# rishikksh20/FastSpeech2

Hardware: AMD Instinct MI355X
Metric: mel-frames/sec (higher is better)
Workload: dtype bf16x3 (FFN conv: f16 x f16 + block-scaled e4m3 cross terms; the decoder's: block-scaled e2m1 cross terms, one E8M0 scale per 16-channel block on both operands); 1 GPU; c3: batch=64 LJSpeech-shape; default.yaml dims, free-running, random-init weights (seed 0), duration bias calibrated to 7.87 frames/phoneme; precision=mix_mx4, utterances=64, phonemes=4528, parallelism=single GPU, launch=eager, device-driven layout (no host sync), overlap_encoder=False, streams=3

## Files before the change

### fastspeech2_amd/csrc/fs2_runtime.hip

```cpp
#include <hip/hip_runtime.h>
#include <dlfcn.h>

#include <algorithm>
#include <cmath>
#include <cstdarg>
#include <cstdio>
#include <cstring>
#include <fstream>
#include <iterator>
#include <list>
#include <map>
#include <string>
#include <type_traits>
#include <vector>

#include "../../include/fs2.h"
#include "attn_bf16.h"
#include "attn_w32.h"
#include "attn_f32.h"
#include "attn_plan.h"
#include "common.h"
#include "elementwise.h"
#include "varshort.h"
#include "layout_rule.h"
#include "layout.h"
#include "gemm_bf16.h"
#include "gemm_plan.h"
#include "gemm_planes.h"
#include "gemm_row4.h"
#include "model_launches.h"
#include "call_plan.h"
#include "gemm_mx.h"
#include "weight_plan.h"
#include "gemm_f32.h"
#include "griffin_lim.h"
#include "gl_pitch.h"
// ... 67 lines not shown
    if (!rf) return false;
    const std::string rec((std::istreambuf_iterator<char>(rf)), std::istreambuf_iterator<char>());
    const size_t k = rec.find("\"so_sha16\"");
    if (k == std::string::npos) return false;
    const size_t q0 = rec.find('"', rec.find(':', k) + 1), q1 = q0 == std::string::npos ? q0 : rec.find('"', q0 + 1);
    if (q1 == std::string::npos) return false;
    const std::string want = rec.substr(q0 + 1, q1 - q0 - 1);
    const size_t c = rec.find("\"clean\"");
    const size_t v = c == std::string::npos ? c : rec.find_first_not_of(" :", c + 7);
    if (v == std::string::npos || rec.compare(v, 4, "true") != 0) return false;
    std::ifstream sf(so, std::ios::binary);
    if (!sf) return false;
    Sha256 sh;
    std::vector<unsigned char> blk(1 << 20);
    while (sf) {
        sf.read(reinterpret_cast<char*>(blk.data()), (std::streamsize)blk.size());
        if (sf.gcount() > 0) sh.update(blk.data(), (size_t)sf.gcount());
    }
    return sh.hex16() == want;
}
bool audit_clean() {
    static const bool ok = audit_clean_of_this_binary();
    return ok;
}

Options& opts() {
    static Options o = [] {
        Options x;
        x.bm = env_int("FS2_BM", -1); x.row8 = env_int("FS2_ROW8", -1); x.qkv8 = env_int("FS2_QKV8", -1);
        x.nosplitk = env_int("FS2_NOSPLITK", 0) != 0; x.f32_rows = env_int("FS2_F32_ROWS", 0) != 0; x.mt8 = env_int("FS2_MT8", -1); x.qkv_split = env_int("FS2_QKV_SPLIT", -1); x.op_att_planes = env_int("FS2_OP_ATT_PLANES", 0); x.fuse_var = env_int("FS2_FUSE_VAR", 1); x.bal = env_int("FS2_BAL", 0); x.w32 = env_int("FS2_ATTN_W32", -1);
        x.row4 = env_int("FS2_ROW4", -1); x.mt4 = env_int("FS2_MT4", -1); x.ffn2_mx = env_int("FS2_FFN2_MX", 1); x.qkv4 = env_int("FS2_QKV4", -1); x.post_mx = env_int("FS2_POST_MX", 1);
        x.tokproj = env_int("FS2_TOKPROJ", 3) & 3; x.tokproj_f32 = env_int("FS2_TOKPROJ_F32", 0) != 0;
        x.varshort = env_int("FS2_VARSHORT", 1) != 0;
        if (!audit_clean()) {
            x.w32 = 0; x.row4 = 0; x.qkv4 = 0;
            fprintf(stderr, "libfs2_hip: no clean ISA-audit record of this binary (libfs2_hip.audit.json next to it): attn_w32 and gemm_row4_bf16 are switched "
                            "off, attn_bf16 / gemm_row8_bf16 run instead; rebuild with `python -c 'import __graft_entry__ as g; g.build()'`\n");
        }
        return x;
    }();
    return o;
}

__global__ void row_l1_bound_kernel(const float* w, const float* b, int N, int K, float xmax, unsigned* out) {
    const int n = blockIdx.x;
    float s = 0.f;
    for (int k = threadIdx.x; k < K; k += blockDim.x) s += fabsf(w[(size_t)n * K + k]);
    for (int o = 32; o > 0; o >>= 1) s += __shfl_xor(s, o);
    __shared__ float part[4];
    if ((threadIdx.x & 63) == 0) part[threadIdx.x >> 6] = s;
    __syncthreads();
    if (threadIdx.x == 0) atomicMax(out, __float_as_uint((part[0] + part[1] + part[2] + part[3]) * xmax + (b ? fabsf(b[n]) : 0.f)));
}
float device_row_l1_bound(hipStream_t s, const float* w, const float* b, int N, int K, float xmax, unsigned* scratch) {
    hipMemsetAsync(scratch, 0, 4, s);
    hipLaunchKernelGGL(row_l1_bound_kernel, dim3(N), dim3(256), 0, s, w, b, N, K, xmax, scratch);
    unsigned u = 0;
    hipMemcpyAsync(&u, scratch, 4, hipMemcpyDeviceToHost, s);
    hipStreamSynchronize(s);
    float f;
    memcpy(&f, &u, 4);
    return f;
}

__global__ void absmax_kernel(const float* x, int64_t n, unsigned* out) {
    float m = 0.f;
// ... 102 lines not shown
inline void allow_lds(const void* kernel, size_t bytes, LdsAttr& st) {
    int dev = 0;
    hipGetDevice(&dev);
    bool& d = st.done[dev & 31];
    if (!d) { hipFuncSetAttribute(kernel, hipFuncAttributeMaxDynamicSharedMemorySize, (int)bytes); d = true; }
}

static_assert(kPlanErrArg == FS2_ERR_ARG && kPlanErrHip == FS2_ERR_HIP && kPlanErrState == FS2_ERR_STATE && kPlanErrUnsupported == FS2_ERR_UNSUPPORTED &&
              kPlanFp32 == FS2_PREC_FP32 && kPlanBf16x3 == FS2_PREC_BF16X3 && kPlanMaxHalo == kMaxHalo && kPlanBN == kB16BN && kPrecMixF16x2 == FS2_PREC_MIX_F16X2 &&
              kPrecMixF16x1 == FS2_PREC_MIX_F16X1 && kPrecMixMx == FS2_PREC_MIX_MX && kPrecMixMx4 == FS2_PREC_MIX_MX4, "gemm_plan.h and model_launches.h restate these");

template <auto K, class A>
hipError_t launch_kernel(dim3 grid, dim3 block, size_t lds, hipStream_t s, const A& a, size_t lds_max = 0) {
    static LdsAttr attr;
    allow_lds(reinterpret_cast<const void*>(K), lds_max ? lds_max : lds, attr);
    hipLaunchKernelGGL(K, grid, block, lds, s, a);
    return hipGetLastError();
}
template <int V> using Int = std::integral_constant<int, V>;
template <int V, int... Vs, typename F>
hipError_t pick(int v, F&& f) {
    if (v == V) return f(Int<V>{});
    if constexpr (sizeof...(Vs) > 0) return pick<Vs...>(v, f);
    else return hipErrorInvalidValue;
}
#define CV(x) decltype(x)::value
constexpr int row4_variant(int epi, int arith, int res) { return epi * 100 + arith * 10 + res; }

template <int NSPLIT, int BM, bool K1, int ARITH>
hipError_t launch_pl(hipStream_t s, const GemmArgs& a, size_t extra_lds = 0) {
    dim3 grid((a.N + kB16BN - 1) / kB16BN, ((a.qk_hi ? a.Rvt : a.R) + BM - 1) / BM, a.ksplit > 1 ? a.ksplit : 1);
    return launch_kernel<gemm_pl_bf16<NSPLIT, BM, K1, ARITH>>(grid, dim3(256), pl_lds_bytes<BM, K1>() + extra_lds, s, a);
}
template <int MT, int EPI, int ARITH, int RES>
hipError_t launch_row4(hipStream_t s, const GemmArgs& a) {
    return launch_kernel<gemm_row4_bf16<3, 3, MT, EPI, 2, ARITH, RES>>(dim3((a.R + 32 * MT - 1) / (32 * MT)), dim3(256), row4_lds_bytes<3, MT>(), s, a);
}

hipError_t run_plan(hipStream_t s, const GemmPlan& p, const GemmArgs& t) {
    switch (p.kernel) {
    case GemmKernel::Row4: {
        auto row4 = [&](auto EPI, auto ARITH, auto RES) { return pick<5, 4>(p.mt, [&](auto MT) { return launch_row4<CV(MT), CV(EPI), CV(ARITH), CV(RES)>(s, t); }); };
        switch (row4_variant(p.epi, p.arith, p.res)) {
        case row4_variant(2, 0, 3): return row4(Int<2>{}, Int<0>{}, Int<3>{});
        case row4_variant(1, 0, 1): return row4(Int<1>{}, Int<0>{}, Int<1>{});
        case row4_variant(4, 0, 1): return row4(Int<4>{}, Int<0>{}, Int<1>{});
        case row4_variant(0, 2, 2): return row4(Int<0>{}, Int<2>{}, Int<2>{});
        case row4_variant(0, 0, 2): return row4(Int<0>{}, Int<0>{}, Int<2>{});
        case row4_variant(0, 0, 1): return row4(Int<0>{}, Int<0>{}, Int<1>{});
        }
        break;
    }
    case GemmKernel::Qkv4:
        return pick<5, 4>(p.mt, [&](auto MT) {
            static_assert((size_t)32 * CV(MT) * kQkvLd * 4 <= row4_lds_bytes<3, CV(MT)>(), "the V pass transposes its tile through the operand ring's memory");
            return launch_kernel<gemm_row4_bf16<3, 3, CV(MT), 3, 2, 0>>(dim3((t.Rvt + 32 * CV(MT) - 1) / (32 * CV(MT)), 3), dim3(256), row4_lds_bytes<3, CV(MT)>(), s, t);
        });
    case GemmKernel::PlMx:
        return pick<160, 192, 224, 256, 128, 64>(p.bm, [&](auto BM) { return launch_pl<1, CV(BM), false, 2>(s, t); });
    case GemmKernel::PlMx4:
        return launch_pl<1, 256, false, 3>(s, t, kMx4RowScaleLds + 2048);
    case GemmKernel::PlF16:
        return pick<3, 2, 1>(p.nsplit, [&](auto NS) {
            return pick<256, 128, 64>(p.bm, [&](auto BM) { return launch_pl<CV(NS), CV(BM), false, 1>(s, t); });
        });
    case GemmKernel::Qkv8:
        return pick<3, 2>(p.nb, [&](auto NB) {
            return pick<3, 1>(p.nsplit, [&](auto NS) {
                return pick<3, 2>(p.mt, [&](auto MT) {
                    return pick<1, 0>(p.apart, [&](auto AP) {
                        const dim3 grid((t.Rvt + 64 * CV(MT) - 1) / (64 * CV(MT)), CV(AP) ? 3 : 1);
                        return launch_kernel<gemm_qkv8_bf16<CV(NS), CV(NB), CV(MT), CV(AP) != 0>>(grid, dim3(512), qkv8_lds_bytes<CV(NB), CV(MT)>(), s, t);
                    });
                });
            });
        });
    case GemmKernel::Row8cTwoLn:
        return pick<3, 1>(p.nsplit, [&](auto NS) { return launch_kernel<gemm_row8c_bf16<CV(NS), 4, 2, 2>>(dim3((t.R + 127) / 128, 1), dim3(512), row8c_lds_bytes<4, 2>(), s, t); });
    case GemmKernel::Row8c:
    case GemmKernel::Row8cGrouped:
        return pick<3, 2>(p.nb, [&](auto NB) {
            return pick<3, 1>(p.nsplit, [&](auto NS) {
                return pick<3, 2>(p.mt, [&](auto MT) {
                    const dim3 grid((t.R + 64 * CV(MT) - 1) / (64 * CV(MT)), t.k_groups > 1 ? t.k_groups : 1);
                    return launch_kernel<gemm_row8c_bf16<CV(NS), CV(NB), CV(MT), 1>>(grid, dim3(512), row8c_lds_bytes<CV(NB), CV(MT)>(), s, t);
                });
            });
        });
    case GemmKernel::Row8:
        return pick<3, 2>(p.nb, [&](auto NB) {
            return pick<3, 1>(p.nsplit, [&](auto NS) {
                return pick<3, 2>(p.mt, [&](auto MT) {
                    const dim3 grid((t.R + 64 * CV(MT) - 1) / (64 * CV(MT)));
// ... 1434 lines not shown

int fs2_op_duration(void* stream, const float* d_log, int64_t n, int64_t* d) {
    if (!d_log || !d || n < 0) return fail(nullptr, FS2_ERR_ARG, "fs2_op_duration: bad arguments");
    if (n == 0) return FS2_OK;
    hipLaunchKernelGGL(duration_kernel, dim3((unsigned)((n + 255) / 256)), dim3(256), 0, (hipStream_t)stream, d_log, n, d);
    hipError_t e = hipGetLastError();
    if (e != hipSuccess) return fail(nullptr, FS2_ERR_HIP, "duration: %s", hipGetErrorString(e));
    return FS2_OK;
}

int fs2_set_option(const char* name, int32_t value) {
    if (!name) return fail(nullptr, FS2_ERR_ARG, "fs2_set_option: null name");
    Options& o = opts();
    const std::string n = name;
    if (n == "FS2_BM") o.bm = value;
    else if (n == "FS2_ROW8") o.row8 = value;
    else if (n == "FS2_QKV8") o.qkv8 = value;
    else if (n == "FS2_NOSPLITK") o.nosplitk = value > 0;
    else if (n == "FS2_F32_ROWS") o.f32_rows = value > 0;
    else if (n == "FS2_MT8") o.mt8 = value;
    else if (n == "FS2_QKV_SPLIT") o.qkv_split = value;
    else if (n == "FS2_OP_ATT_PLANES") o.op_att_planes = value;
    else if (n == "FS2_FUSE_VAR") o.fuse_var = value != 0;
    else if (n == "FS2_BAL") o.bal = value < 0 ? 0 : value;
    else if (n == "FS2_ATTN_W32") o.w32 = value;
    else if (n == "FS2_ROW4") o.row4 = value;
    else if (n == "FS2_MT4") o.mt4 = value;
    else if (n == "FS2_FFN2_MX") o.ffn2_mx = value != 0;
    else if (n == "FS2_QKV4") o.qkv4 = value;
    else if (n == "FS2_POST_MX") o.post_mx = value != 0;
    else if (n == "FS2_TOKPROJ") o.tokproj = value < 0 ? 3 : (value & 3);
    else if (n == "FS2_TOKPROJ_F32") o.tokproj_f32 = value > 0;
    else if (n == "FS2_VARSHORT") o.varshort = value != 0;
    else return fail(nullptr, FS2_ERR_ARG, "fs2_set_option: unknown option %s", name);
    return FS2_OK;
}

int fs2_get_option(const char* name, int32_t* value) {
    if (!name || !value) return fail(nullptr, FS2_ERR_ARG, "fs2_get_option: null argument");
    const Options& o = opts();
    const std::string n = name;
    if (n == "FS2_AUDIT_CLEAN") *value = audit_clean() ? 1 : 0;
    else if (n == "attn_w32_active") *value = o.w32 != 0;
    else if (n == "row4_active") *value = o.row4 != 0;
    else if (n == "qkv4_active") *value = o.qkv4 != 0 && o.row4 != 0;
    else if (n == "FS2_BM") *value = o.bm;
    else if (n == "FS2_ROW8") *value = o.row8;
    else if (n == "FS2_QKV8") *value = o.qkv8;
    else if (n == "FS2_NOSPLITK") *value = o.nosplitk;
    else if (n == "FS2_F32_ROWS") *value = o.f32_rows;
    else if (n == "FS2_MT8") *value = o.mt8;
    else if (n == "FS2_QKV_SPLIT") *value = o.qkv_split;
    else if (n == "FS2_OP_ATT_PLANES") *value = o.op_att_planes;
    else if (n == "FS2_FUSE_VAR") *value = o.fuse_var;
    else if (n == "FS2_BAL") *value = o.bal;
    else if (n == "FS2_ATTN_W32") *value = o.w32;
    else if (n == "FS2_ROW4") *value = o.row4;
    else if (n == "FS2_MT4") *value = o.mt4;
    else if (n == "FS2_FFN2_MX") *value = o.ffn2_mx;
    else if (n == "FS2_QKV4") *value = o.qkv4;
    else if (n == "FS2_POST_MX") *value = o.post_mx;
    else if (n == "FS2_TOKPROJ") *value = o.tokproj;
    else if (n == "FS2_TOKPROJ_F32") *value = o.tokproj_f32;
    else if (n == "FS2_VARSHORT") *value = o.varshort;
    else return fail(nullptr, FS2_ERR_ARG, "fs2_get_option: unknown option %s", name);
    return FS2_OK;
}

int fs2_get_counter(fs2_handle* h, void* stream, const char* name, int64_t* value, int32_t reset) {
    if (!h || !name || !value) return fail(h, FS2_ERR_ARG, "fs2_get_counter: null argument");
    if (std::string(name) != "attn_slow_path_waves") return fail(h, FS2_ERR_ARG, "fs2_get_counter: unknown counter %s", name);
    DeviceGuard g(h->cfg.device);
    HIP_TRY(h, g.err);
    hipStream_t s = (hipStream_t)stream;
    int v = 0;
    HIP_TRY(h, hipMemcpyAsync(&v, h->counters, sizeof(int), hipMemcpyDeviceToHost, s));
    if (reset) HIP_TRY(h, hipMemsetAsync(h->counters, 0, sizeof(int), s));
    HIP_TRY(h, hipStreamSynchronize(s));
    *value = v;
    return FS2_OK;
}

int fs2_op_bucketize(void* stream, const float* x, int64_t n, const float* bins, int32_t nb, int32_t* idx) {
    if (!x || !bins || !idx || n < 0) return fail(nullptr, FS2_ERR_ARG, "fs2_op_bucketize: bad arguments");
    if (n == 0) return FS2_OK;
    hipLaunchKernelGGL(bucketize_kernel, dim3((unsigned)((n + 255) / 256)), dim3(256), 0, (hipStream_t)stream, x, n, bins, nb, idx);
    hipError_t e = hipGetLastError();
    if (e != hipSuccess) return fail(nullptr, FS2_ERR_HIP, "bucketize: %s", hipGetErrorString(e));
    return FS2_OK;
}

size_t fs2_op_vocode_workspace_bytes(int32_t B, const int32_t* lens) { return fs2_op_vocode_workspace_bytes_geom(kGlNfft, kGlHop, kGlNfft, 80, B, lens); }

size_t fs2_op_vocode_workspace_bytes_geom(int32_t n_fft, int32_t hop, int32_t win, int32_t n_mels, int32_t B, const int32_t* lens) {
    return gl_workspace_bytes({"fs2_op_vocode_workspace_bytes_geom", GlKind::Synthesis, {n_fft, hop, win, n_mels}, gl_host_batch(B, nullptr, lens)});
}

// ... 208 lines not shown
```

### fastspeech2_amd/csrc/gemm_plan.h

```cpp
#pragma once
#include <algorithm>

#include "gemm_args.h"

namespace fs2 {

constexpr int kPlanErrArg = -1, kPlanErrHip = -2, kPlanErrState = -3, kPlanErrUnsupported = -6;
constexpr int kPlanFp32 = 0, kPlanBf16x3 = 1;
constexpr int kPlanMaxHalo = 16;
constexpr int kPlanBN = 128;

struct Options {
    int bm = -1;
    int bal = 0;
    int row8 = -1;
    int qkv8 = -1;
    int nosplitk = 0;
    int f32_rows = 0;
    int fuse_var = 1;
    int mt8 = -1;
    int op_att_planes = 0;
    int qkv_split = -1;
    int w32 = -1;
    int row4 = -1;
    int mt4 = -1;
    int qkv4 = -1;
    int ffn2_mx = 1;
    int post_mx = 1;
    int tokproj = 3;
    int tokproj_f32 = 0;
    int varshort = 1;
};

constexpr int kSplitRegime = 8192, kSplitRows = 16384;
constexpr int kCus = 256;

inline bool row_regime(long regime_rows, int forced) { return forced >= 0 ? forced != 0 : (regime_rows + 127) / 128 >= 128; }

inline long rows_in_use(const GemmArgs& a, long rows) { return a.regime_rows > 0 ? std::min<long>(rows, a.regime_rows) : rows; }

inline int row8_mt(long rows, int wgs = 1) {
    const long t128 = (rows + 127) / 128, t192 = (rows + 191) / 192;
    if (t128 > kCus && t192 <= kCus) return 3;
    return (wgs > 1 && t128 * wgs > kCus && t192 * wgs <= kCus) ? 3 : 2;
}

inline int row4_mt(long rows) {
    const long r4 = ((rows + 127) / 128 + kCus - 1) / kCus * 128, r5 = ((rows + 159) / 160 + kCus - 1) / kCus * 160;
    return r5 <= r4 ? 5 : 4;
}
inline int row4_epi(const GemmArgs& a) {
    if (a.ktaps != 1 || a.N != 384 || !a.ln_g || a.Y || !a.Yp || a.resid || a.relu_pre || a.dot_w || a.k_groups > 1 || a.ln_groups > 1 || a.qk_hi || a.yp_col_off) return -1;
    if (a.Cpad % 64 != 0 || a.yp_chunks * 32 != a.N) return -1;
    if (a.residp && a.residp_chunks * 32 != a.N) return -1;
    if (a.pe) return (a.act_post == 1 && a.yp_f16 == 0 && !a.residp) ? 2 : -1;
    if (a.act_post != 0 || !a.residp) return -1;
    if (a.yp_f16 == 2) return a.residp_mx ? -1 : 1;
    if (a.yp_f16 == 3) return (a.residp_mx || !a.yp_rowscale) ? -1 : 4;
    return a.yp_f16 == 0 ? 0 : -1;
}

inline void qkv8_plan(long rows, const Options& o, int& mt, int& apart) {
    double best = 1e30;
    for (int m = 2; m <= 3; ++m)
// ... 12 lines not shown
}

inline bool use_qkv8(const GemmArgs& a, const Options& o) {
    if (!a.qk_hi || a.ktaps != 1 || (a.att_D != 256 && a.att_D != 384) || a.N != 3 * a.att_D) return false;
    return row_regime(a.regime_rows ? a.regime_rows : a.Rvt, o.qkv8);
}

inline bool use_row8(const GemmArgs& a, const Options& o) {
    const int Ng = a.k_groups > 1 ? a.N / a.k_groups : a.N;
    const bool two_ln_groups = a.ln_groups == 2 && a.k_groups <= 1 && a.N == 512 && a.ktaps > 1;
    if (a.qk_hi || (!two_ln_groups && Ng != 256 && Ng != 384)) return false;
    if (a.ln_groups > 1 && !two_ln_groups && a.ln_groups != a.k_groups) return false;
    if (a.ktaps > 1) {
        if (!a.ln_g || a.pe || a.f16_terms) return false;
    } else if (a.dot_w || !(a.ln_g || a.pe) || a.k_groups > 1 || a.ln_groups > 1) return false;
    return row_regime(a.regime_rows ? a.regime_rows : a.R, o.row8);
}

inline int conv_bm_balanced(long rows, long nN) {
    const long ypr = std::max<long>(1, 2 * kCus / nN);
    const long rounds = std::max<long>(1, (rows + 256 * ypr - 1) / (256 * ypr));
    const long h = (rows + rounds * ypr - 1) / (rounds * ypr);
    return (int)std::min<long>(256, std::max<long>(160, (h + 31) / 32 * 32));
}
inline int conv_bm(const GemmArgs& a, int arith, int nsplit, int ksplit, const Options& o) {
    const int force = o.bm > 0 ? o.bm : 0;
    const long rows = a.R, nN = (a.N + kPlanBN - 1) / kPlanBN;
    int bm = force ? force : (nN * ((rows + 255) / 256) >= 512 ? 256 : (nN * ((rows + 127) / 128) >= 400 ? 128 : 64));
    if (arith == 1) return bm == 256 ? 256 : (bm == 128 ? 128 : 64);
    if (bm <= 128) return bm == 128 ? 128 : 64;
    if (arith == 0 && nsplit != 3) return 256;
    if (!force && o.bal && (arith == 2 || ksplit <= 1)) bm = conv_bm_balanced(o.bal == 2 ? rows : rows_in_use(a, rows), nN);
    return bm <= 160 ? 160 : (bm <= 192 ? 192 : (bm <= 224 ? 224 : 256));
}

inline int pick_ksplit(const GemmArgs& a, long rr, int max_extra_splits, bool own_y, size_t ld) {
    const int nchunks = a.Cpad / 32;
    const long wgs = (long)((a.N + kPlanBN - 1) / kPlanBN) * ((rr + 63) / 64);
    for (int cand = 4; cand >= 2; --cand)
        if (nchunks % cand == 0 && (nchunks / cand) * a.ktaps >= 4 && wgs * cand <= 1024 && cand - 1 <= max_extra_splits &&
            (size_t)(cand - (own_y ? 1 : 0)) * a.R * ld <= a.kpart_cap) return cand;
    return 1;
}

inline bool rows_supported(int N) { return N == 80 || N == 256 || N == 384; }

enum class GemmKernel {
    None,
    RowsF32,
    TileF32,
    TileRowsF32,
    PlBf16,
    PlF16,
    PlMx,
    PlMx4,
    Row8,
    Row8c,
    Row8cGrouped,
    Row8cTwoLn,
    Row4,
    Qkv8,
    Qkv4,
};
enum class RowsOut { None, Y, Scratch, KpartSlab };

struct GemmPlan {
    GemmKernel kernel = GemmKernel::None;
    int nsplit = 0, nb = 0;
    int bm = 0, mt = 0;
    bool k1 = false;
    int apart = 0, epi = -1, arith = 0, res = 0;
    int ksplit = 1;
    RowsOut y = RowsOut::None;
    bool build_planes = false;
    bool rows_pass = false;
    int err = 0;
    const char* msg = nullptr;
    int m0 = 0, m1 = 0;
    int tile_rows() const { return bm ? bm : (kernel == GemmKernel::Row4 || kernel == GemmKernel::Qkv4 ? 32 : 64) * mt; }
};
inline GemmPlan refused(int err, const char* msg, int m0 = 0, int m1 = 0) {
    GemmPlan p;
    p.err = err; p.msg = msg; p.m0 = m0; p.m1 = m1;
    return p;
}

inline GemmPlan plan_gemm(const GemmArgs& a, int precision, const Options& o) {
    if (a.ktaps - 1 > kPlanMaxHalo) return refused(kPlanErrUnsupported, "%s: kernel size %d > %d", a.ktaps, kPlanMaxHalo + 1);
    if (a.C % 4 != 0 || a.ldx % 4 != 0) return refused(kPlanErrUnsupported, "%s: channels %d / ld %d must be multiples of 4", a.C, a.ldx);
    const bool need_rows = a.ln_g || a.dot_w || a.pe;
    GemmPlan p;
    if (precision == kPlanFp32) {
        if (need_rows && a.N >= 128 && a.N <= 1024 && a.N % 4 == 0 && (a.Y || a.scratch) && !o.f32_rows) {
            p.kernel = GemmKernel::TileRowsF32; p.rows_pass = true;
            p.y = a.Y ? RowsOut::Y : RowsOut::Scratch;
        } else if (need_rows || (a.N < 128 && rows_supported(a.N))) {
            if (!rows_supported(a.N)) return refused(kPlanErrUnsupported, "%s: row-epilogue GEMM needs N in {80,256,384}, got %d", a.N);
            p.kernel = GemmKernel::RowsF32; p.nb = a.N == 80 ? 5 : (a.N == 256 ? 16 : 24);
            p.y = a.Y ? RowsOut::Y : RowsOut::None;
        } else {
            p.kernel = GemmKernel::TileF32; p.y = RowsOut::Y;
        }
        return p;
// ... 7 lines not shown
    const int epi = (row8 && x3 && o.row4 != 0) ? row4_epi(a) : -1;
    if ((a.residp || (need_rows && !a.Y && a.Yp && !a.dot_w && a.ktaps == 1 && !a.scratch)) && epi < 0)
        return refused(kPlanErrState, "%s: a planes-only launch (residual as planes / no fp32 rows) exists on gemm_row4_bf16 only and this one would not run there");
    if (a.yp_col_off && !(row8 && a.ktaps > 1)) return refused(kPlanErrUnsupported, "%s: a plane column offset exists in the row-complete conv kernel only");
    if (a.Yp && a.yp_chunks * 32 >= a.N + 32 && !(row8 && a.ktaps > 1))
        return refused(kPlanErrUnsupported, "%s: planes %d columns wide from a launch of %d: filling a slice of a plane row exists in the row-complete conv kernel only", a.yp_chunks * 32, a.N);
    const bool y_needed = (need_rows && !row8) || (!a.Yp && !a.qk_hi && !(row8 && a.dot_w));
    p.y = a.Y ? RowsOut::Y : ((y_needed && a.scratch) ? RowsOut::Scratch : RowsOut::None);
    if (y_needed && p.y == RowsOut::None) return refused(kPlanErrArg, "%s: no output or scratch buffer");
    if (a.qk_hi && (a.ktaps != 1 || a.att_D % kPlanBN != 0 || a.N != 3 * a.att_D)) return refused(kPlanErrUnsupported, "%s: fused QKV split needs D %% 128 == 0");
    const long rr = a.regime_rows ? a.regime_rows : a.R;
    if (!row8 && !a.qk_hi && a.kpart && !o.nosplitk && a.N <= 1024 && rr <= kSplitRegime && a.R <= kSplitRows && a.mx != 2) {
        const bool own_y = p.y != RowsOut::None;
        p.ksplit = pick_ksplit(a, rr, a.ksplit, own_y, p.y == RowsOut::Y ? (size_t)a.ldy : (size_t)a.N);
        if (p.ksplit > 1 && !own_y) p.y = RowsOut::KpartSlab;
    }
    p.rows_pass = (need_rows && !row8) || p.ksplit > 1;
    const bool mx_row4 = a.mx && a.ktaps == 1 && epi == 0 && a.Cpad % 128 == 0 && a.Xp;
    if ((a.f16_terms || a.mx) && !mx_row4 && (a.ktaps == 1 || need_rows || a.qk_hi)) return refused(kPlanErrUnsupported, "%s: the fp16 arithmetic exists for plain convolutions only");
    if (a.mx && !mx_row4 && (a.ktaps < 3 || a.C % 128 != 0 || a.N % 128 != 0)) return refused(kPlanErrUnsupported, "%s: the mx arithmetic needs a convolution with C %% 128 == 0 and N %% 128 == 0");
    if (a.mx == 2 && (!a.x_rowscale || !a.w_rowscale || !a.Xp || p.ksplit > 1)) return refused(kPlanErrState, "%s: the mx4 arithmetic needs mx4 planes with their row scales and the weight image's channel scales");
    p.build_planes = !a.Xp;
    p.nsplit = x3 ? 3 : 1;
    const int mt8 = (o.mt8 > 0 ? o.mt8 : row8_mt(rows_in_use(a, a.R), a.k_groups > 1 ? a.k_groups : 1)) >= 3 ? 3 : 2;
    const bool force_mt4 = o.mt4 == 4 || o.mt4 == 5;
    if (mx_row4 || epi >= 0) {
        if (a.mx && !a.residp_mx) return refused(kPlanErrHip, "%s launch: invalid argument");
        p.kernel = GemmKernel::Row4; p.epi = epi; p.arith = a.mx ? 2 : 0;
        p.res = epi == 2 ? 3 : ((epi == 0 && a.residp_mx) ? 2 : 1);
        p.mt = force_mt4 ? o.mt4 : row4_mt(rows_in_use(a, a.R));
    } else if (a.mx == 2) {
        if (a.Cpad != 384) return refused(kPlanErrHip, "%s launch: invalid argument");
        p.kernel = GemmKernel::PlMx4; p.nsplit = 1; p.arith = 3; p.bm = 256;
    } else if (a.mx) {
        p.kernel = GemmKernel::PlMx; p.nsplit = 1; p.arith = 2; p.bm = conv_bm(a, 2, 1, p.ksplit, o);
    } else if (a.f16_terms) {
        p.kernel = GemmKernel::PlF16; p.nsplit = a.f16_terms == 3 ? 3 : (a.f16_terms == 2 ? 2 : 1); p.arith = 1; p.bm = conv_bm(a, 1, p.nsplit, p.ksplit, o);
    } else if (use_qkv8(a, o)) {
        if (x3 && o.qkv4 != 0 && o.row4 != 0 && a.att_D == 384 && a.Cpad % 64 == 0) {
            p.kernel = GemmKernel::Qkv4; p.epi = 3; p.mt = force_mt4 ? o.mt4 : qkv4_mt(rows_in_use(a, a.Rvt));
        } else {
            p.kernel = GemmKernel::Qkv8; p.nb = a.att_D == 384 ? 3 : 2; p.mt = 2;
            qkv8_plan(rows_in_use(a, a.Rvt), o, p.mt, p.apart);
        }
    } else if (row8 && a.ktaps > 1 && a.ln_groups == 2 && a.k_groups <= 1) {
        p.kernel = GemmKernel::Row8cTwoLn; p.nb = 4; p.mt = 2;
    } else if (row8 && a.ktaps > 1) {
        p.kernel = a.k_groups > 1 ? GemmKernel::Row8cGrouped : GemmKernel::Row8c;
        p.nb = (a.k_groups > 1 ? a.N / a.k_groups : a.N) == 384 ? 3 : 2; p.mt = mt8;
    } else if (row8) {
        p.kernel = GemmKernel::Row8; p.nb = a.N == 384 ? 3 : 2; p.mt = mt8;
    } else {
        p.kernel = GemmKernel::PlBf16; p.k1 = a.ktaps == 1;
        p.bm = p.k1 ? (o.bm == 128 ? 128 : 64)
                    : conv_bm(a, 0, p.nsplit, p.ksplit, o);
    }
    return p;
}

}
```

### fastspeech2_amd/csrc/gemm_planes.h

```cpp
#pragma once
#include <type_traits>
#include "gemm_bf16.h"

namespace fs2 {

template <int BM, bool K1> constexpr int pl_arows() { return K1 ? BM : BM + kMaxHalo; }
template <int BM, bool K1>
constexpr size_t pl_lds_bytes() {
    const size_t ops = (size_t)(K1 ? 2 : 1) * pl_arows<BM, K1>() * 128 + 2 * (size_t)kB16BN * 128;
    const size_t out = (K1 && BM <= 128) ? (size_t)BM * kQkvLd * 4 : 0;
    return ops > out ? ops : out;
}
typedef __attribute__((address_space(3))) const unsigned short lds_u16_t;
constexpr int kMx4ScLd = 24;
constexpr int kMx4RowScaleLds = 272 * kMx4ScLd;
template <int BM, bool K1> constexpr int pl_occ() { return pl_lds_bytes<BM, K1>() > 53 * 1024 ? 2 : 3; }

__global__ void to_planes(const float* __restrict__ X, int ldx, int C, int R, int nchunks, void* __restrict__ Xp, int f16 = 0, float scale = 1.f) {
    const int64_t i = (int64_t)blockIdx.x * blockDim.x + threadIdx.x;
    const int per_row = nchunks * 8;
    if (i >= (int64_t)R * per_row) return;
    const int row = (int)(i / per_row), c = (int)(i - (int64_t)row * per_row) * 4;
    f32x4 v = f32x4{0.f, 0.f, 0.f, 0.f};
    if (c < C) v = *reinterpret_cast<const f32x4*>(X + (size_t)row * ldx + c);
// ... 275 lines not shown
                    uint2 hi, lo;
                    split4(f32x4{acc[mt][0][r], acc[mt][1][r], acc[mt][2][r], acc[mt][3][r]} * f, hi, lo);
                    const size_t off = (size_t)row * 2 * a.att_D + col;
                    *reinterpret_cast<uint2*>(qkh + off) = hi;
                    *reinterpret_cast<uint2*>(qkl + off) = lo;
                }
            return;
        }
        if (a.qk_hi != nullptr) {
            float* tile = reinterpret_cast<float*>(smem_p);
            __syncthreads();
#pragma unroll
            for (int mt = 0; mt < MT; ++mt)
#pragma unroll
                for (int r = 0; r < 4; ++r)
                {
                    const int trow = wm * (BM / 2) + mt * 16 + rperm(lg * 4 + r);
                    *reinterpret_cast<f32x4*>(tile + trow * kQkvLd + ((wn * 64 + 4 * lr) ^ qkv_tile_swz(trow))) =
                        f32x4{acc[mt][0][r], acc[mt][1][r], acc[mt][2][r], acc[mt][3][r]};
                }
            __syncthreads();
            vt_tile_store<BM>(a, tile, m0, n0, tid);
            return;
        }
    }
    if (ks > 0) {
        GemmArgs p = a;
        p.Y = a.kpart + (size_t)(ks - 1) * a.kpart_stride;
        p.Yp = nullptr; p.relu_pre = 0; p.act_post = 0;
        pl_epilogue<MT>(p, acc, m0 + wm * (BM / 2), col, lg);
        return;
    }
    pl_epilogue<MT>(a, acc, m0 + wm * (BM / 2), col, lg);
}

}

namespace fs2 {

template <int NSPLIT, int MT, int NT>
__device__ __forceinline__ void row8_mfma_step(const char* Bs, int nrow, int lg, const bf16x8_t (&ah)[MT], const bf16x8_t (&al)[MT], f32x4 (&acc)[MT][NT]) {
    constexpr int kReads = NSPLIT == 3 ? 4 : 2, kMfma = 2 * MT * NSPLIT;
    const char* bp0 = Bs + swz(nrow, lg);
    const char* bp1 = Bs + swz(nrow, 4 + lg);
    bf16x8_t bh[2][2], bl[2][2];
#pragma unroll
    for (int u = 0; u < 2; ++u) {
        bh[0][u] = *reinterpret_cast<const bf16x8_t*>(bp0 + u * 2048);
        if (NSPLIT == 3) bl[0][u] = *reinterpret_cast<const bf16x8_t*>(bp1 + u * 2048);
    }
    __builtin_amdgcn_sched_group_barrier(0x100, kReads, 0);
#pragma unroll
    for (int n2 = 0; n2 < NT; n2 += 2) {
        const int cb = (n2 >> 1) & 1, nb = cb ^ 1;
        if (n2 + 2 < NT) {
#pragma unroll
            for (int u = 0; u < 2; ++u) {
                bh[nb][u] = *reinterpret_cast<const bf16x8_t*>(bp0 + (n2 + 2 + u) * 2048);
                if (NSPLIT == 3) bl[nb][u] = *reinterpret_cast<const bf16x8_t*>(bp1 + (n2 + 2 + u) * 2048);
            }
            __builtin_amdgcn_sched_group_barrier(0x100, kReads, 0);
        }
        __builtin_amdgcn_sched_group_barrier(0x008, kMfma, 0);
        if (NSPLIT == 3) {
#pragma unroll
            for (int u = 0; u < 2; ++u)
// ... 585 lines not shown
```

Before: 10.29 million mel-frames/s.

## Add paired-tile MX conv GEMM kernel sharing weight stages across two row tiles

```diff
diff --git a/fastspeech2_amd/csrc/fs2_runtime.hip b/fastspeech2_amd/csrc/fs2_runtime.hip
--- a/fastspeech2_amd/csrc/fs2_runtime.hip
+++ b/fastspeech2_amd/csrc/fs2_runtime.hip
@@ -2,6 +2,7 @@
 #include <dlfcn.h>
 
 #include <algorithm>
+#include <atomic>
 #include <cmath>
 #include <cstdarg>
 #include <cstdio>
@@ -135,6 +136,7 @@
         x.row4 = env_int("FS2_ROW4", -1); x.mt4 = env_int("FS2_MT4", -1); x.ffn2_mx = env_int("FS2_FFN2_MX", 1); x.qkv4 = env_int("FS2_QKV4", -1); x.post_mx = env_int("FS2_POST_MX", 1);
         x.tokproj = env_int("FS2_TOKPROJ", 3) & 3; x.tokproj_f32 = env_int("FS2_TOKPROJ_F32", 0) != 0;
         x.varshort = env_int("FS2_VARSHORT", 1) != 0;
+        x.conv_pair = env_int("FS2_CONV_PAIR", -1);
         if (!audit_clean()) {
             x.w32 = 0; x.row4 = 0; x.qkv4 = 0;
             fprintf(stderr, "libfs2_hip: no clean ISA-audit record of this binary (libfs2_hip.audit.json next to it): attn_w32 and gemm_row4_bf16 are switched "
@@ -303,6 +305,13 @@
     dim3 grid((a.N + kB16BN - 1) / kB16BN, ((a.qk_hi ? a.Rvt : a.R) + BM - 1) / BM, a.ksplit > 1 ? a.ksplit : 1);
     return launch_kernel<gemm_pl_bf16<NSPLIT, BM, K1, ARITH>>(grid, dim3(256), pl_lds_bytes<BM, K1>() + extra_lds, s, a);
 }
+std::atomic<int> g_conv_pair_launches{0};
+template <int ARITH>
+hipError_t launch_pair(hipStream_t s, const GemmArgs& a) {
+    const int tiles = (a.R + 255) / 256;
+    g_conv_pair_launches.fetch_add(1, std::memory_order_relaxed);
+    return launch_kernel<gemm_pl_pair<ARITH>>(dim3((a.N + kB16BN - 1) / kB16BN, (tiles + 1) / 2), dim3(512), pl_pair_lds_bytes<ARITH>(), s, a);
+}
 template <int MT, int EPI, int ARITH, int RES>
 hipError_t launch_row4(hipStream_t s, const GemmArgs& a) {
     return launch_kernel<gemm_row4_bf16<3, 3, MT, EPI, 2, ARITH, RES>>(dim3((a.R + 32 * MT - 1) / (32 * MT)), dim3(256), row4_lds_bytes<3, MT>(), s, a);
@@ -328,8 +337,10 @@
             return launch_kernel<gemm_row4_bf16<3, 3, CV(MT), 3, 2, 0>>(dim3((t.Rvt + 32 * CV(MT) - 1) / (32 * CV(MT)), 3), dim3(256), row4_lds_bytes<3, CV(MT)>(), s, t);
         });
     case GemmKernel::PlMx:
+        if (p.pair) return launch_pair<2>(s, t);
         return pick<160, 192, 224, 256, 128, 64>(p.bm, [&](auto BM) { return launch_pl<1, CV(BM), false, 2>(s, t); });
     case GemmKernel::PlMx4:
+        if (p.pair) return launch_pair<3>(s, t);
         return launch_pl<1, 256, false, 3>(s, t, kMx4RowScaleLds + 2048);
     case GemmKernel::PlF16:
         return pick<3, 2, 1>(p.nsplit, [&](auto NS) {
@@ -1830,6 +1841,7 @@
     else if (n == "FS2_TOKPROJ") o.tokproj = value < 0 ? 3 : (value & 3);
     else if (n == "FS2_TOKPROJ_F32") o.tokproj_f32 = value > 0;
     else if (n == "FS2_VARSHORT") o.varshort = value != 0;
+    else if (n == "FS2_CONV_PAIR") o.conv_pair = value;
     else return fail(nullptr, FS2_ERR_ARG, "fs2_set_option: unknown option %s", name);
     return FS2_OK;
 }
@@ -1861,6 +1873,8 @@
     else if (n == "FS2_TOKPROJ") *value = o.tokproj;
     else if (n == "FS2_TOKPROJ_F32") *value = o.tokproj_f32;
     else if (n == "FS2_VARSHORT") *value = o.varshort;
+    else if (n == "FS2_CONV_PAIR") *value = o.conv_pair;
+    else if (n == "conv_pair_launches") *value = g_conv_pair_launches.load(std::memory_order_relaxed);
     else return fail(nullptr, FS2_ERR_ARG, "fs2_get_option: unknown option %s", name);
     return FS2_OK;
 }
diff --git a/fastspeech2_amd/csrc/gemm_plan.h b/fastspeech2_amd/csrc/gemm_plan.h
--- a/fastspeech2_amd/csrc/gemm_plan.h
+++ b/fastspeech2_amd/csrc/gemm_plan.h
@@ -30,6 +30,7 @@
     int tokproj = 3;
     int tokproj_f32 = 0;
     int varshort = 1;
+    int conv_pair = -1;
 };
 
 constexpr int kSplitRegime = 8192, kSplitRows = 16384;
@@ -108,6 +109,12 @@
     if (arith == 0 && nsplit != 3) return 256;
     if (!force && o.bal && (arith == 2 || ksplit <= 1)) bm = conv_bm_balanced(o.bal == 2 ? rows : rows_in_use(a, rows), nN);
     return bm <= 160 ? 160 : (bm <= 192 ? 192 : (bm <= 224 ? 224 : 256));
+}
+
+inline bool conv_pair_regime(long regime_rows, long nN) { return nN * (((regime_rows + 255) / 256 + 1) / 2) >= kCus; }
+inline bool conv_pair(const GemmArgs& a, int arith, int bm, int ksplit, const Options& o) {
+    if (o.conv_pair == 0 || (arith != 2 && arith != 3) || bm != 256 || ksplit != 1 || a.ktaps <= 1 || a.k_groups > 1 || a.qk_hi) return false;
+    return o.conv_pair > 0 || conv_pair_regime(a.regime_rows ? a.regime_rows : a.R, (a.N + kPlanBN - 1) / kPlanBN);
 }
 
 inline int pick_ksplit(const GemmArgs& a, long rr, int max_extra_splits, bool own_y, size_t ld) {
@@ -145,6 +152,7 @@
     int nsplit = 0, nb = 0;
     int bm = 0, mt = 0;
     bool k1 = false;
+    bool pair = false;
     int apart = 0, epi = -1, arith = 0, res = 0;
     int ksplit = 1;
     RowsOut y = RowsOut::None;
@@ -218,8 +226,10 @@
     } else if (a.mx == 2) {
         if (a.Cpad != 384) return refused(kPlanErrHip, "%s launch: invalid argument");
         p.kernel = GemmKernel::PlMx4; p.nsplit = 1; p.arith = 3; p.bm = 256;
+        p.pair = conv_pair(a, p.arith, p.bm, p.ksplit, o);
     } else if (a.mx) {
         p.kernel = GemmKernel::PlMx; p.nsplit = 1; p.arith = 2; p.bm = conv_bm(a, 2, 1, p.ksplit, o);
+        p.pair = conv_pair(a, p.arith, p.bm, p.ksplit, o);
     } else if (a.f16_terms) {
         p.kernel = GemmKernel::PlF16; p.nsplit = a.f16_terms == 3 ? 3 : (a.f16_terms == 2 ? 2 : 1); p.arith = 1; p.bm = conv_bm(a, 1, p.nsplit, p.ksplit, o);
     } else if (use_qkv8(a, o)) {
diff --git a/fastspeech2_amd/csrc/gemm_planes.h b/fastspeech2_amd/csrc/gemm_planes.h
--- a/fastspeech2_amd/csrc/gemm_planes.h
+++ b/fastspeech2_amd/csrc/gemm_planes.h
@@ -331,6 +331,244 @@
         return;
     }
     pl_epilogue<MT>(a, acc, m0 + wm * (BM / 2), col, lg);
+}
+
+template <int ARITH> constexpr size_t pl_pair_lds_bytes() {
+    return (size_t)2 * pl_arows<256, false>() * 128 + (size_t)3 * kB16BN * 128 + (ARITH == 3 ? (size_t)2 * kMx4RowScaleLds + 3 * 1024 : 0);
+}
+
+__device__ __forceinline__ void pair_wait_barrier(int n) {
+    if (n == 3) asm volatile("s_waitcnt vmcnt(3) lgkmcnt(0)\n\ts_barrier" ::: "memory");
+    else if (n == 2) asm volatile("s_waitcnt vmcnt(2) lgkmcnt(0)\n\ts_barrier" ::: "memory");
+    else asm volatile("s_waitcnt vmcnt(0) lgkmcnt(0)\n\ts_barrier" ::: "memory");
+}
+
+template <int ARITH>
+__global__ __launch_bounds__(512, 1) void gemm_pl_pair(GemmArgs a) {
+    static_assert(ARITH == 2 || ARITH == 3, "the paired form exists in the mx arithmetics");
+    constexpr bool MX4 = ARITH == 3;
+    constexpr int BM = 256, MT = BM / 32, AROWS = pl_arows<BM, false>();
+    constexpr unsigned kAbytes = AROWS * 128, kBoff = 2 * kAbytes, kStage = kB16BN * 128, kScOff = kBoff + 3 * kStage, kSbOff = kScOff + 2 * kMx4RowScaleLds;
+    extern __shared__ __attribute__((aligned(16))) char smem_p[];
+    const int tid = threadIdx.x, lane = tid & 63;
+    const int wave = __builtin_amdgcn_readfirstlane(tid >> 6);
+    const int half = wave >> 2, w4 = wave & 3;
+    const int wm = w4 >> 1, wn = w4 & 1;
+    const int n0 = blockIdx.x * kB16BN, m0 = (2 * blockIdx.y + half) * BM;
+    const int rlim = a.Rp != nullptr ? ((*a.Rp + 127) & ~127) : 0x7fffffff;
+    if ((int)(2 * blockIdx.y) * BM >= rlim) return;
+    const bool live = m0 < a.R && m0 < rlim;
+    const int ktaps = a.ktaps;
+    const int P = (ktaps - 1) >> 1;
+    const int lr = lane & 15, lg = lane >> 4;
+    const int lp = rperm(lr);
+    const __bf16* Wb = reinterpret_cast<const __bf16*>(a.W);
+    const __bf16* Xp = reinterpret_cast<const __bf16*>(a.Xp);
+    const int xunits = a.Cpad / 32;
+    const int nchunks = MX4 ? xunits - xunits / 4 : xunits;
+    const int it_end = nchunks * ktaps;
+    const int jrow = lane >> 3, jslot = lane & 7;
+
+    char* As = smem_p + half * kAbytes;
+    const char* Bs0 = smem_p + kBoff;
+    const unsigned lds0 = __builtin_amdgcn_readfirstlane((unsigned)(size_t)(lds_void_t*)smem_p);
+    const int a_instr = (BM + 2 * P + 7) >> 3;
+    const int sA = jslot ^ (jrow >> 1) ^ ((w4 & 1) << 2);
+    const int arow0 = m0 - P + w4 * 8 + jrow;
+    const int xrc = a.xp_row_chunks ? a.xp_row_chunks : xunits;
+    const __bf16* a_src0 = Xp + (ptrdiff_t)arow0 * xrc * 64 + sA * 8;
+    const size_t a_qstride = (size_t)32 * xrc * 64;
+    const unsigned ldsA = lds0 + half * kAbytes + w4 * 1024;
+    auto dma_A = [&](int ch) {
+        unsigned dst = ldsA;
+        const __bf16* src = a_src0 + (size_t)ch * 64;
+        int row = arow0;
+        for (int q = w4; q < a_instr; q += 4) {
+            const bool ok = row >= 0 && row < a.R;
+            const void* sp = ok ? static_cast<const void*>(src) : static_cast<const void*>(g_zero16);
+            dma16(sp, dst);
+            dst += 4096; src += a_qstride; row += 32;
+        }
+    };
+    const int jB = (wave & 1) * 8 + jrow;
+    const int sB = jslot ^ ((jB >> 1) & 7);
+    const __bf16* b_src0 = Wb + ((size_t)(n0 + 4 * rperm_inv(jB) + (wave >> 1)) * it_end) * 64 + sB * 8;
+    const size_t b_o2 = (size_t)64 * it_end * 64;
+    const unsigned ldsB = lds0 + kBoff + wave * 1024;
+    const int it_cross0 = (xunits >> 1) * ktaps;
+    const unsigned char* wsb_tile = MX4 ? a.w_rowscale + (size_t)blockIdx.x * (xunits / 4) * ktaps * 1024 + lane * 16 : nullptr;
+    auto dma_stage = [&](int it, int rb) {
+        const __bf16* src = b_src0 + (size_t)it * 64;
+        const unsigned dst = ldsB + rb * kStage;
+        dma16(src, dst);
+        dma16(src + b_o2, dst + 8192);
+        if (MX4 && wave == 0 && it >= it_cross0) dma16(wsb_tile + (size_t)(it - it_cross0) * 1024, lds0 + kSbOff + rb * 1024);
+    };
+    auto stage_count = [&](int it) { return it < it_end ? 2 + ((MX4 && wave == 0 && it >= it_cross0) ? 1 : 0) : 0; };
+
+    unsigned char* Sc = reinterpret_cast<unsigned char*>(smem_p) + kScOff + half * kMx4RowScaleLds;
+    constexpr int sc_ld = kMx4ScLd;
+    const unsigned char* Sb0 = reinterpret_cast<const unsigned char*>(smem_p) + kSbOff;
+    const unsigned sc_lane = lds0 + kScOff + half * kMx4RowScaleLds + (unsigned)((wm * (BM / 2) + lp) * sc_ld + lg * 2);
+    if constexpr (MX4) {
+        static_assert(AROWS * kMx4ScLd <= kMx4RowScaleLds, "row-scale records of the A tile");
+        constexpr int ncu = kMx4ScLd / 8;
+        if (live)
+            for (int t = tid & 255; t < AROWS * ncu; t += 256) {
+                const int rt = t / ncu, u = t - rt * ncu, row = m0 - P + rt;
+                *reinterpret_cast<uint2*>(Sc + rt * sc_ld + u * 8) =
+                    (row >= 0 && row < a.R) ? *reinterpret_cast<const uint2*>(a.x_rowscale + (size_t)row * 32 + u * 8) : uint2{0x7f7f7f7fu, 0x7f7f7f7fu};
+            }
+    }
+    if (live) dma_A(0);
+    dma_stage(0, 0);
+    if (1 < it_end) dma_stage(1, 1);
+
+    const int col = n0 + wn * 64 + 4 * lr;
+    const int row_base = m0 + wm * (BM / 2);
+    unsigned vmask = 0;
+    if (live) {
+        const int* __restrict__ rpos = a.row_pos;
+        int pv[MT][4];
+#pragma unroll
+        for (int mt = 0; mt < MT; ++mt)
+#pragma unroll
+            for (int r = 0; r < 4; ++r) {
+                const int row = row_base + mt * 16 + rperm(lg * 4 + r);
+                pv[mt][r] = loadi_or_zero(rpos + row, (rpos != nullptr) & (row < a.R));
+            }
+#pragma unroll
+        for (int mt = 0; mt < MT; ++mt)
+#pragma unroll
+            for (int r = 0; r < 4; ++r) {
+                const int row = row_base + mt * 16 + rperm(lg * 4 + r);
+                vmask |= ((unsigned)(row < a.R) & (unsigned)(pv[mt][r] >= 0)) << (mt * 4 + r);
+            }
+    }
+    f32x4 acc[MT][4];
+    {
+        f32x4 bv = f32x4{0.f, 0.f, 0.f, 0.f};
+        if (a.bias && col < a.N) bv = *reinterpret_cast<const f32x4*>(a.bias + col);
+#pragma unroll
+        for (int mt = 0; mt < MT; ++mt)
+#pragma unroll
+            for (int r = 0; r < 4; ++r) {
+                const int row = row_base + mt * 16 + rperm(lg * 4 + r);
+                f32x4 v = bv;
+                v += load4_or_zero(a.resid + (size_t)row * a.ldr + col, a.resid != nullptr && live && row < a.R && col < a.N);
+#pragma unroll
+                for (int nt = 0; nt < 4; ++nt) acc[mt][nt][r] = v[nt];
+            }
+    }
+    int it = 0, rb = 0;
+#ifdef FS2_GEMM_TIMING
+    long long tprev = __builtin_readcyclecounter();
+    const long long t_begin = tprev, r_begin = __builtin_amdgcn_s_memrealtime();
+#endif
+    auto k_loop = [&](auto kind_tag, const int cb, const int ce) {
+        constexpr int KIND = decltype(kind_tag)::value;
+        for (int chunk = cb; chunk < ce; ++chunk) {
+            for (int tap = 0; tap < ktaps; ++tap, ++it) {
+                pair_wait_barrier(stage_count(it + 1));
+                FS2_GT(0)
+                const bool refill = tap == ktaps - 1 && chunk + 1 < nchunks;
+                const int rb2 = rb == 0 ? 2 : rb - 1;
+                if (!refill && it + 2 < it_end) dma_stage(it + 2, rb2);
+                FS2_GT(1)
+                if (live) {
+                    const char* Bs = Bs0 + rb * kStage;
+                    bf16x8_t b0[4], b1[4];
+#pragma unroll
+                    for (int nt = 0; nt < 4; ++nt) {
+                        const int n = wn * 64 + nt * 16 + lp;
+                        b0[nt] = *reinterpret_cast<const bf16x8_t*>(Bs + swz(n, lg));
+                        b1[nt] = *reinterpret_cast<const bf16x8_t*>(Bs + swz(n, 4 + lg));
+                    }
+                    const unsigned scp = sc_lane + (unsigned)__builtin_amdgcn_readfirstlane(tap * sc_ld + (chunk - (xunits >> 1)) * 8);
+                    int2 sbq = int2{0, 0};
+                    if constexpr (KIND == 3) sbq = *reinterpret_cast<const int2*>(Sb0 + rb * 1024 + (lg * 128 + wn * 64 + 4 * lr) * 2);
+                    if (FS2_SETPRIO) __builtin_amdgcn_s_setprio(1);
+                    const int rbase = wm * (BM / 2) + lp + tap;
+                    const char* ap0 = As + (rbase << 7) + ((lg ^ ((rbase >> 1) & 7)) << 4);
+                    const char* ap1 = As + (rbase << 7) + (((4 + lg) ^ ((rbase >> 1) & 7)) << 4);
+#pragma unroll
+                    for (int mt = 0; mt < MT; ++mt) {
+                        const bf16x8_t a0 = *reinterpret_cast<const bf16x8_t*>(ap0 + mt * 2048);
+                        const bf16x8_t a1 = *reinterpret_cast<const bf16x8_t*>(ap1 + mt * 2048);
+                        if constexpr (KIND == 3) {
+                            const int sa = *reinterpret_cast<lds_u16_t*>(scp + (unsigned)(mt * 16 * sc_ld));
+                            const v4i_t z4 = v4i_t{0, 0, 0, 0};
+                            const v8i_t av0 = __builtin_shufflevector(__builtin_bit_cast(v4i_t, a0), z4, 0, 1, 2, 3, 4, 5, 6, 7);
+                            const v8i_t av1 = __builtin_shufflevector(__builtin_bit_cast(v4i_t, a1), z4, 0, 1, 2, 3, 4, 5, 6, 7);
+#define FS2_MX4_PAIR(NT_)                                                                                                                              \
+                            acc[mt][NT_] = __builtin_amdgcn_mfma_scale_f32_16x16x128_f8f6f4(av0, __builtin_shufflevector(__builtin_bit_cast(v4i_t, b0[NT_]), z4, 0, 1, 2, 3, 4, 5, 6, 7), \
+                                                                                           acc[mt][NT_], 4, 4, 0, sa, 2 * ((NT_) & 1), (NT_) < 2 ? sbq.x : sbq.y);
+                            FS2_MX4_PAIR(0) FS2_MX4_PAIR(1) FS2_MX4_PAIR(2) FS2_MX4_PAIR(3)
+#undef FS2_MX4_PAIR
+#define FS2_MX4_PAIR(NT_)                                                                                                                              \
+                            acc[mt][NT_] = __builtin_amdgcn_mfma_scale_f32_16x16x128_f8f6f4(av1, __builtin_shufflevector(__builtin_bit_cast(v4i_t, b1[NT_]), z4, 0, 1, 2, 3, 4, 5, 6, 7), \
+                                                                                           acc[mt][NT_], 4, 4, 1, sa, 2 * ((NT_) & 1) + 1, (NT_) < 2 ? sbq.x : sbq.y);
+                            FS2_MX4_PAIR(0) FS2_MX4_PAIR(1) FS2_MX4_PAIR(2) FS2_MX4_PAIR(3)
+#undef FS2_MX4_PAIR
+                        } else if constexpr (KIND == 2) {
+                            const v8i_t av = __builtin_shufflevector(__builtin_bit_cast(v4i_t, a0), __builtin_bit_cast(v4i_t, a1), 0, 1, 2, 3, 4, 5, 6, 7);
+#pragma unroll
+                            for (int nt = 0; nt < 4; ++nt) {
+                                const v8i_t bv = __builtin_shufflevector(__builtin_bit_cast(v4i_t, b0[nt]), __builtin_bit_cast(v4i_t, b1[nt]), 0, 1, 2, 3, 4, 5, 6, 7);
+                                acc[mt][nt] = __builtin_amdgcn_mfma_scale_f32_16x16x128_f8f6f4(av, bv, acc[mt][nt], 0, 0, 0, a.mx_scale, 0, a.mx_scale_b);
+                            }
+                        } else {
+#pragma unroll
+                            for (int nt = 0; nt < 4; ++nt) acc[mt][nt] = mfma16<true>(a0, b0[nt], acc[mt][nt]);
+#pragma unroll
+                            for (int nt = 0; nt < 4; ++nt) acc[mt][nt] = mfma16<true>(a1, b1[nt], acc[mt][nt]);
+                        }
+                    }
+                    if (FS2_SETPRIO) __builtin_amdgcn_s_setprio(0);
+                }
+                FS2_GT(2)
+                if (refill) {
+                    asm volatile("s_waitcnt lgkmcnt(0)\n\ts_barrier" ::: "memory");
+                    if (live) dma_A(chunk + 1);
+                    if (it + 2 < it_end) dma_stage(it + 2, rb2);
+                    FS2_GT(3)
+                }
+                rb = rb == 2 ? 0 : rb + 1;
+            }
+        }
+    };
+    const int nmain = MX4 ? xunits >> 1 : nchunks >> 1;
+    k_loop(std::integral_constant<int, 1>{}, 0, nmain);
+    k_loop(std::integral_constant<int, MX4 ? 3 : 2>{}, nmain, nchunks);
+#ifdef FS2_GEMM_TIMING
+    if (blockIdx.x == 0 && blockIdx.y == 0 && threadIdx.x == 0) {
+        g_gemm_phase[6] = __builtin_readcyclecounter() - t_begin;
+        g_gemm_phase[7] = __builtin_amdgcn_s_memrealtime() - r_begin;
+    }
+#endif
+    if (!live) return;
+    float* __restrict__ Y = a.Y;
+    void* __restrict__ Yp = a.Yp;
+    const bool colok = col < a.N;
+    const bool pcol = Yp != nullptr && col < a.yp_chunks * 32;
+    const bool relu_first = a.relu_pre != 0;
+#pragma unroll
+    for (int mt = 0; mt < MT; ++mt)
+#pragma unroll
+        for (int r = 0; r < 4; ++r) {
+            const int row = row_base + mt * 16 + rperm(lg * 4 + r);
+            const bool inb = row < a.R, valid = (vmask >> (mt * 4 + r)) & 1u;
+            f32x4 v;
+#pragma unroll
+            for (int j = 0; j < 4; ++j) {
+                float t = acc[mt][j][r];
+                if (relu_first) t = fmaxf(t, 0.f);
+                t = apply_act(t, a.act_post);
+                v[j] = (valid && colok) ? t : 0.f;
+            }
+            if (Y && inb && colok) *reinterpret_cast<f32x4*>(Y + (size_t)row * a.ldy + col) = v;
+            if (pcol && inb) store_planes4m(Yp, row, a.yp_chunks, col, v, a.yp_f16, a.yp_scale);
+        }
 }
 
 }
```

After: 10.17 million mel-frames/s. 1.2% lower.
